# mbortolon97/6dgs

Hardware: AMD Instinct MI355X
Metric: poses/sec (higher is better)
Workload: dtype f32

## Files before the change

### 6dgs_amd/_lib.py

```python
from __future__ import annotations

import ctypes as C
import os

_HERE = os.path.dirname(os.path.abspath(__file__))
LIB_PATH = os.path.join(_HERE, "csrc", "lib6dgs_hip.so")
if os.environ.get("SIXDGS_LIB"):
    LIB_PATH = os.path.abspath(os.environ["SIXDGS_LIB"])

vp = C.c_void_p
i64 = C.c_int64
i32 = C.c_int
sz = C.c_size_t


PROFILE_SLOTS = 128
ABI_VERSION = 10


class Profile(C.Structure):
    _fields_ = [("count", i32), ("start", vp * PROFILE_SLOTS), ("stop", vp * PROFILE_SLOTS),
                ("flops", C.c_double * PROFILE_SLOTS), ("bytes", C.c_double * PROFILE_SLOTS)]


# ... 21 lines not shown
    "sixdgs_splat_views": (i32, [vp, vp, i32, vp, vp, i32, i32, i64, vp, i32, i32, i32, i32, C.c_float, C.c_float, vp, vp, vp, vp, sz, vp]),
    "sixdgs_packed_weights_floats": (sz, []),
    "sixdgs_pack_weights": (i32, [vp] * 13 + [C.POINTER(ScorerWeights), vp]),
    "sixdgs_ray_encode": (i32, [vp, vp, vp, i64, vp, vp]),
    "sixdgs_ray_keys_workspace_bytes": (sz, [i64, i64]),
    "sixdgs_ray_keys": (i32, [vp, vp, vp, i64, C.POINTER(ScorerWeights), vp, vp, vp, sz, vp]),
    "sixdgs_ray_keys_ex": (i32, [vp, vp, vp, i64, C.POINTER(ScorerWeights), vp, vp, vp, vp, vp, vp, sz, vp, C.POINTER(Profile), i32]),
    "sixdgs_key_planes_f16_bytes": (sz, [i64]),
    "sixdgs_split_planes_f16": (i32, [vp, i64, i64, vp, vp, vp]),
    "sixdgs_score_pass1": (i32, [vp, vp, vp, i32, vp, vp, vp, i64, i32, vp, vp, sz, vp, C.POINTER(Profile), i32]),
    "sixdgs_score_pass2": (i32, [vp, vp, i32, i32, i64, i32, vp, vp, vp, vp, sz, vp, i32]),
    "sixdgs_score_backward_workspace_bytes": (sz, [i32]),
    "sixdgs_score_backward": (i32, [vp, vp, i32, vp, i64, vp, vp, vp, vp, vp, sz, vp]),
    "sixdgs_score_backward_split_workspace_bytes": (sz, [i32, i64, i32]),
    "sixdgs_score_backward_split": (i32, [vp, vp, i32, vp, i64, vp, vp, vp, vp, i32, vp, sz, vp]),
    "sixdgs_score_topk_ex": (i32, [vp, vp, vp, i32, vp, vp, vp, i64, i32, vp, vp, vp, vp, vp, sz, vp, C.POINTER(Profile), i32]),
    "sixdgs_score_select_workspace_bytes": (sz, [i64, i32, i32, i32]),
    "sixdgs_score_select": (i32, [vp, vp, vp, i32, vp, vp, vp, i64, vp, vp, i64, i32, i32, vp, vp, vp, vp, sz, vp, C.POINTER(Profile)]),
    "sixdgs_tok_attention": (i32, [vp, i64, i32, i32, i32, vp, i64, vp]),
    "sixdgs_im2col": (i32, [vp, i64, i64, i64, i64, i32, i32, i32, i32, i32, i32, vp, vp]),
    "sixdgs_u8_to_planar": (i32, [vp, i32, i64, vp, vp, vp]),
    "sixdgs_image_prep": (i32, [vp, i32, i32, i32, vp, i32, i32, i32, i32, i32, vp, vp, vp, vp]),
    "sixdgs_tok_pack_bytes": (sz, [i32, i32]),
    "sixdgs_tok_pack": (i32, [vp, i32, i32, i64, vp, vp, vp]),
    "sixdgs_tok_linear": (i32, [vp, i64, i32, i64, i32, vp, vp, C.c_float, vp, vp, vp, i32, i32, vp, i64, vp, vp, i64, vp]),
    "sixdgs_key_planes_norm_max": (i32, [vp, vp, i64, vp, vp]),
    "sixdgs_select_workspace_bytes": (sz, [i64, i32, i32, i32]),
    "sixdgs_select_candidates_workspace_bytes": (sz, [i64, i32, i32, i32]),
    "sixdgs_select_begin": (i32, [vp, vp, vp, i32, vp, vp, i64, i64, vp, vp, vp, sz, vp]),
    "sixdgs_select_sweep_plan": (i32, [vp, i32, vp, vp, i32]),
    "sixdgs_select_sweep": (i32, [vp, vp, vp, i32, vp, vp, i64, vp, vp, vp, i64, vp, vp, sz, vp, C.POINTER(Profile)]),
    "sixdgs_select_candidates": (i32, [vp, i64, i64, vp, vp, vp, i32, vp, vp, vp, i32, i32, vp, vp, vp, sz, vp]),
    "sixdgs_select_rescore": (i32, [vp, vp, i32, vp, vp, i32, vp, vp, vp, vp, i64, i32, i32, i32, vp, vp, vp, vp, sz, vp]),
    "sixdgs_select_sample_stats": (i32, [vp, vp, vp, i32, vp, vp, i64, vp, vp, sz, vp]),
    "sixdgs_select_prepare": (i32, [vp, vp, i32, i64, i64, vp, vp, vp]),
    "sixdgs_select_topk_u": (i32, [vp, i64, i64, vp, i32, i32, vp, vp, sz, vp]),
    "sixdgs_linear_splitk_workspace_bytes": (sz, [i64, i32, i32]),
    "sixdgs_linear_splitk": (i32, [vp, i64, i32, i64, vp, i64, vp, i32, i32, vp, i64, i32, vp, sz, vp, i32]),
    "sixdgs_linear_ex": (i32, [vp, i64, i32, i64, vp, i64, vp, i32, i32, vp, i64, vp, i32]),
    "sixdgs_profile_collect": (i32, [C.POINTER(Profile), C.POINTER(C.c_double), C.POINTER(C.c_double), C.POINTER(C.c_double),
                                    C.POINTER(i32)]),
    "sixdgs_linear": (i32, [vp, i64, i32, i64, vp, i64, vp, i32, i32, vp, i64, vp]),
    "sixdgs_q_proj": (i32, [vp, vp, i32, C.POINTER(ScorerWeights), vp, vp]),
    "sixdgs_score_topk_workspace_bytes": (sz, [i64, i32, i32]),
    "sixdgs_score_topk_workspace_bytes_ex": (sz, [i64, i32, i32, i32, i32]),
    "sixdgs_score_topk": (i32, [vp, vp, i32, vp, i64, i32, vp, vp, vp, vp, vp, sz, vp]),
    "sixdgs_topk_workspace_bytes": (sz, [i64, i32, i32]),
    "sixdgs_topk": (i32, [vp, i64, i32, i32, vp, vp, vp, sz, vp]),
    "sixdgs_distance_target_workspace_bytes": (sz, [i64]),
    "sixdgs_distance_target": (i32, [vp, vp, i64, vp, i32, vp, vp, vp, sz, vp]),
    "sixdgs_solve_pose": (i32, [vp, vp, i64, vp, vp, i32, vp, vp, i32, vp, vp, vp, vp, vp, vp, vp]),
    "sixdgs_solve_pose_consensus_workspace_bytes": (sz, [i32, i32]),
    "sixdgs_solve_pose_consensus": (i32, [vp, vp, i64, vp, vp, i32, vp, vp, i32, C.c_float, i32] + [vp] * 10 + [vp, sz, vp]),
}

_lib = None


def load():
    global _lib
    if _lib is not None:
        return _lib
    import torch

    if not os.path.exists(LIB_PATH):
        raise RuntimeError(
# ... 24 lines not shown
```

### 6dgs_amd/csrc/score.hip

```cpp
#include <stdlib.h>

#include <cstdlib>
#include <cstdio>
#include "gemm_kernel.h"
#include "sweep_plan.h"
#include "sweep_layout.h"

using namespace sdg;

namespace {

constexpr int kT = SIXDGS_MAX_TOKENS;
constexpr float kSqrtD = 19.595917942265423f;

struct LogitsArgs {
  const float* q;
  const int* n_tok;
  const float* key;
  float* logits;
  float* partial;
  int64_t r, ldl;
  int tiles_per_group, n_tiles, n_groups;
  int b0;
};
// ... 1207 lines not shown
    if (i + 2 < R) m = fmaxf(m, a.z);
    if (i + 3 < R) m = fmaxf(m, a.w);
  }
  if (tmax != nullptr) {
    m = sdg_wave_max(m);
    const int64_t tile = (i - 4 * sdg_lane()) >> 8;
    if (sdg_lane() == 0 && tile * 256 < R) tmax[(int64_t)img * tmax_stride + tile] = m;
  }
}

__global__ void __launch_bounds__(256) k_plane_norm_max(const char* __restrict__ planes, const float* __restrict__ inv_scale, int64_t rows,
                                                        unsigned* __restrict__ out) {
  const int lane = sdg_lane();
  const int64_t wave0 = (int64_t)blockIdx.x * 4 + sdg_wave(), nw = (int64_t)gridDim.x * 4;
  float best = 0.f;
  for (int64_t row = wave0; row < rows; row += nw) {
    float ss = 0.f;
    if (lane < 48) {
      const char* p = planes + row * kRowF + (lane >> 2) * kSlabF + (lane & 3) * 16;
      const f16x8 h = *reinterpret_cast<const f16x8*>(p), l = *reinterpret_cast<const f16x8*>(p + 64);
#pragma unroll
      for (int e = 0; e < 8; ++e) {
        const float x = (float)h[e] + (float)l[e];
        ss = __builtin_fmaf(x, x, ss);
      }
    }
    ss = sdg_wave_sum(ss);
    best = fmaxf(best, sqrtf(ss) * inv_scale[row >> 7]);
  }
  if (lane == 0 && best > 0.f) atomicMax(out, __float_as_uint(best * 1.000244140625f));
}

constexpr float kEpsPerX = 1.4e-4f, kEpsConst = 1.3e-5f;
__global__ void __launch_bounds__(kT) k_sel_bounds(const float* __restrict__ gsum, const int* __restrict__ n_tok, const float* __restrict__ valU,
                                                   const float* __restrict__ q, const float* __restrict__ key_norm_max, int topk, int k_eff,
                                                   float* __restrict__ info, const int* __restrict__ only) {
  __shared__ float smin[4], smax[4], sq[4];
  const int bl = blockIdx.x, t = threadIdx.x, M = n_tok[bl];
  if (only != nullptr && only[bl] == 0) return;
  const float g = gsum[(int64_t)bl * kT + t];
  float lo = t < M ? g : INFINITY, hi = t < M ? g : -INFINITY;
  bool bad = t < M && !(g > 0.f && g < INFINITY);
  float qn = 0.f;
  if (t < M) {
    const float4* qr = reinterpret_cast<const float4*>(q + ((int64_t)bl * kT + t) * SIXDGS_D);
    float ss = 0.f;
    for (int i = 0; i < SIXDGS_D / 4; ++i) {
      const float4 v = qr[i];
      ss = __builtin_fmaf(v.x, v.x, ss); ss = __builtin_fmaf(v.y, v.y, ss); ss = __builtin_fmaf(v.z, v.z, ss); ss = __builtin_fmaf(v.w, v.w, ss);
    }
    qn = sqrtf(ss) * 1.000244140625f;
  }
#pragma unroll
  for (int o = 32; o > 0; o >>= 1) {
    lo = fminf(lo, __shfl_xor(lo, o, 64));
    hi = fmaxf(hi, __shfl_xor(hi, o, 64));
    qn = fmaxf(qn, __shfl_xor(qn, o, 64));
  }
  const unsigned long long anybad = __ballot(bad);
  if (sdg_lane() == 0) { smin[sdg_wave()] = anybad ? NAN : lo; smax[sdg_wave()] = hi; sq[sdg_wave()] = qn; }
  __syncthreads();
  if (t == 0) {
    float flag = 0.f, thr = INFINITY, eps = 0.f, x = 0.f;
    if (M <= 0) flag = 1.f;
    else {
      float a = smin[0], b = smax[0], qm = sq[0];
      bool nan = a != a;
      for (int w = 1; w < 4; ++w) { nan = nan || smin[w] != smin[w]; a = fminf(a, smin[w]); b = fmaxf(b, smax[w]); qm = fmaxf(qm, sq[w]); }
      const float uk = valU[(int64_t)bl * topk + (k_eff - 1)];
      x = qm * key_norm_max[0] * kInvSqrtD * 1.0000002f;
      eps = x * kEpsPerX + kEpsConst;
      if (nan || !(uk >= 0.f && uk < INFINITY) || !(a > 0.f) || !(eps < 0.25f)) flag = 2.f;
      else thr = (uk * (a / b)) * ((1.f - eps) / (1.f + eps)) * 0.9999998f;
    }
    info[bl * 4 + 0] = thr;
    info[bl * 4 + 1] = flag;
    info[bl * 4 + 2] = eps;
    info[bl * 4 + 3] = x;
  }
}

__global__ void k_sel_need_exact(const int* __restrict__ total, const float* __restrict__ info, int nb, int cmax, int* __restrict__ need) {
  const int bl = blockIdx.x * blockDim.x + threadIdx.x;
  if (bl >= nb) return;
  need[bl] = (info[bl * 4 + 1] == 0.f && total[bl] > cmax) ? 1 : 0;
}

__global__ void k_sel_count(const int* __restrict__ total, const float* __restrict__ info, int nb, int* __restrict__ d_count) {
  const int bl = blockIdx.x * blockDim.x + threadIdx.x;
  if (bl >= nb) return;
  const float flag = info[bl * 4 + 1];
  d_count[bl] = flag == 1.f ? -2 : (flag != 0.f ? -1 : total[bl]);
}

template <bool WRITE>
__global__ void __launch_bounds__(256) k_sel_candidates(const float* __restrict__ U, int64_t stride, int64_t R, const float* __restrict__ info,
                                                        int64_t span, unsigned* __restrict__ counts, const unsigned* __restrict__ offs,
                                                        int64_t* __restrict__ cand, int cmax, const int* __restrict__ only,
                                                        const float* __restrict__ tmax_all) {
  __shared__ int sc[4];
  const int bl = blockIdx.y;
  if (only != nullptr && only[bl] == 0) return;
  const float thr = info[bl * 4 + 0];
  const float* u = U + (int64_t)bl * stride;
  const float* tmax = tmax_all ? tmax_all + (int64_t)bl * (stride >> 8) : nullptr;
  const int64_t i0 = (int64_t)blockIdx.x * span, i1 = min(i0 + span, R);
  unsigned run = 0;
  const unsigned base = WRITE ? offs[(int64_t)bl * gridDim.x + blockIdx.x] : 0u;
  for (int64_t c0 = i0; c0 < i1; c0 += 256) {
    if (tmax != nullptr && !(tmax[c0 >> 8] >= thr)) continue;
    const int64_t i = c0 + threadIdx.x;
    const bool in = i < i1 && u[i] >= thr;
// ... 65 lines not shown
    }
#pragma unroll
    for (int c = 0; c < 8; ++c) {
      double a = acc[c];
#pragma unroll
      for (int j = 0; j < 4; ++j) {
        const f16x8 kh = *reinterpret_cast<const f16x8*>(krow[c] + sl * kSlabF + j * 16);
        const f16x8 kl = *reinterpret_cast<const f16x8*>(krow[c] + sl * kSlabF + 64 + j * 16);
#pragma unroll
        for (int e = 0; e < 8; ++e) {
          const double h = (double)(float)kh[e], l = (double)(float)kl[e], qhh = (double)(float)qh[j][e], qll = (double)(float)ql[j][e];
          a = __builtin_fma(h, qll, a);
          a = __builtin_fma(l, qhh, a);
          a = __builtin_fma(h, qhh, a);
        }
      }
      acc[c] = a;
    }
  }
  const float cq = qinv[2 * b + (t >> 7)], ct = t < M ? ctok[(int64_t)bl * kT + t] : -INFINITY;
  const float gt = gsum[(int64_t)bl * kT + t], rgt = (t < M && gt > 0.f) ? 1.f / gt : 0.f;
#pragma unroll
  for (int c = 0; c < 8; ++c) {
    const float cfl = ((cq * kscale[c]) * kInvSqrtD) * kLog2e;
    float e = t < M ? __builtin_amdgcn_exp2f(__builtin_fmaf((float)acc[c], cfl, ct)) * rgt : 0.f;
    e = sdg_wave_sum(e);
    if (sdg_lane() == 0) red[c][sdg_wave()] = e;
  }
  __syncthreads();
  if (t < 8 && c0 + t < cmax)
    cscore[(int64_t)bl * cmax + c0 + t] = t < nc ? (red[t][0] + red[t][1]) + (red[t][2] + red[t][3]) : -INFINITY;
}

__global__ void __launch_bounds__(1024) k_sel_emit(const int64_t* __restrict__ lidx, const float* __restrict__ lval, const int64_t* __restrict__ cand,
                                                   const int* __restrict__ count, int cmax, int topk, int k_eff, int allow_fewer,
                                                   int64_t* __restrict__ idx, float* __restrict__ val, int* __restrict__ status) {
  const int bl = blockIdx.x, j = threadIdx.x;
  const int n = count[bl];
  int st = n;
  if (n == -2) st = 0;
  else if (n < 0 || n > cmax || (n < k_eff && !allow_fewer)) st = -1;
  if (allow_fewer && n >= 0 && n < k_eff) k_eff = n;
  if (j == 0) status[bl] = st;
  if (j >= topk) return;
  if (n == -2) {
    idx[(int64_t)bl * topk + j] = j < k_eff ? j : -1;
    val[(int64_t)bl * topk + j] = j < k_eff ? 0.f : NAN;
  } else if (st < 0 || j >= k_eff) {
    idx[(int64_t)bl * topk + j] = -1;
    val[(int64_t)bl * topk + j] = NAN;
  } else {
    idx[(int64_t)bl * topk + j] = cand[(int64_t)bl * cmax + lidx[(int64_t)bl * topk + j]];
    val[(int64_t)bl * topk + j] = lval[(int64_t)bl * topk + j];
  }
}

constexpr int64_t kTopkSmallMax = 1 << 17;
__global__ void __launch_bounds__(1024) k_topk_small(const float* __restrict__ scores, int64_t stride, int n, int topk, int k_eff,
                                                      int64_t* __restrict__ idx, float* __restrict__ val, const int* __restrict__ only) {
  __shared__ unsigned hist[256];
  __shared__ unsigned sel[3];
  __shared__ unsigned slot;
  __shared__ unsigned sk[1024];
  __shared__ long long si[1024];
  __shared__ int wc[2][16];
  const int b = blockIdx.x, t = threadIdx.x, lane = t & 63, wv = t >> 6;
  if (only != nullptr && only[b] == 0) return;
  const float* s = scores + (int64_t)b * stride;
  sk[t] = 0u;
  si[t] = 0x7fffffffffffffffll;
  unsigned prefix = 0u, remain = (unsigned)k_eff;
  if (k_eff > 0) {
    for (int p = 0; p < 4; ++p) {
      if (t < 256) hist[t] = 0u;
      __syncthreads();
      const unsigned hi_mask = p == 0 ? 0u : (0xffffffffu << (32 - 8 * p));
      const int shift = 24 - 8 * p;
      for (int c0 = 0; c0 < n; c0 += 8 * 1024) {
        float v8[8];
#pragma unroll
        for (int u = 0; u < 8; ++u) {
          const int i = c0 + u * 1024 + t;
          v8[u] = i < n ? s[i] : 0.f;
        }
#pragma unroll
        for (int u = 0; u < 8; ++u) {
          const int i = c0 + u * 1024 + t;
          if (c0 + u * 1024 >= n) break;
          unsigned key = 0u;
          bool act = false;
          if (i < n) {
            key = score_key(v8[u]);
            act = (key & hi_mask) == prefix;
          }
          const unsigned bin = (key >> shift) & 255u;
          const unsigned long long m = __ballot(act);
          if (m != 0ull) {
            const int leader = __ffsll((long long)m) - 1;
            const unsigned lb = (unsigned)__shfl((int)bin, leader);
            const unsigned long long same = __ballot(act && bin == lb);
            if (lane == leader) atomicAdd(&hist[lb], (unsigned)__popcll(same));
// ... 80 lines not shown
        if (w2 < wv) { og += g; oe += e; }
        tg += g;
        te += e;
      }
      __syncthreads();
      const unsigned long long below = (1ull << lane) - 1ull;
      if (gt) {
        const unsigned pos = run_g + og + (unsigned)__popcll(bg & below);
        if (pos < 1024u) { sk[pos] = key; si[pos] = (long long)i; }
      } else if (eq) {
        const unsigned re = run_e + oe + (unsigned)__popcll(be & below);
        if (re < remain && n_greater + re < 1024u) { sk[n_greater + re] = key; si[n_greater + re] = (long long)i; }
      }
      run_g += tg;
      run_e += te;
      if (run_e >= remain && run_g >= n_greater) break;
    }
    }
  }
  __syncthreads();
  for (int size = 2; size <= 1024; size <<= 1)
    for (int strd = size >> 1; strd > 0; strd >>= 1) {
      const int p = t ^ strd;
      if (p > t) {
        const bool up = (t & size) == 0;
        const unsigned ka = sk[t], kb = sk[p];
        const long long ia = si[t], ib = si[p];
        const bool a_first = ka > kb || (ka == kb && ia < ib);
        if (up ? !a_first : a_first) { sk[t] = kb; sk[p] = ka; si[t] = ib; si[p] = ia; }
      }
      __syncthreads();
    }
  if (t < topk) {
    if (t < k_eff) { idx[(int64_t)b * topk + t] = si[t]; val[(int64_t)b * topk + t] = key_score(sk[t]); }
    else { idx[(int64_t)b * topk + t] = -1; val[(int64_t)b * topk + t] = NAN; }
  }
}

struct TopkPlan {
  int nb;
  int64_t span;
  size_t off_hist, off_counts, off_offs, off_ckey, off_cidx, bytes;
};
TopkPlan topk_plan(int64_t r, int batch, int topk) {
  TopkPlan p;
  int64_t nb = sdg_cdiv(r, 256 * 16);
  if (nb > 2048) nb = 2048;
  if (nb < 1) nb = 1;
  p.nb = (int)nb;
  p.span = sdg_cdiv(sdg_cdiv(r, nb), 256) * 256;
  if (p.span < 256) p.span = 256;
  size_t o = 0;
  p.off_hist = o;   o += sdg_align((size_t)batch * 4 * 256 * sizeof(unsigned));
  p.off_counts = o; o += sdg_align((size_t)batch * nb * 2 * sizeof(unsigned));
  p.off_offs = o;   o += sdg_align((size_t)batch * nb * 2 * sizeof(unsigned));
  p.off_ckey = o;   o += sdg_align((size_t)batch * topk * sizeof(unsigned));
  p.off_cidx = o;   o += sdg_align((size_t)batch * topk * sizeof(int64_t));
  p.bytes = o;
  return p;
}

int run_topk(const float* scores, int64_t stride, int64_t r, int batch, int topk, int64_t* idx, float* val, char* ws,
             hipStream_t s, const int* only = nullptr) {
  const TopkPlan p = topk_plan(r, batch, topk);
  unsigned* hist = (unsigned*)(ws + p.off_hist);
  unsigned* counts = (unsigned*)(ws + p.off_counts);
  unsigned* offs = (unsigned*)(ws + p.off_offs);
  unsigned* ckey = (unsigned*)(ws + p.off_ckey);
  int64_t* cidx = (int64_t*)(ws + p.off_cidx);
// ... 570 lines not shown
  if (!tiles) {
    hipLaunchKernelGGL(k_sel_candidates<false>, cg, dim3(256), 0, s, u, u_stride, r, w.info, w.p.span, w.counts, w.offs, cand, max_candidates, none, u_tile_max);
    hipLaunchKernelGGL(k_sel_scan, dim3((unsigned)batch), dim3(1024), 0, s, w.counts, w.p.nbc, w.offs, w.total);
    hipLaunchKernelGGL(k_sel_candidates<true>, cg, dim3(256), 0, s, u, u_stride, r, w.info, w.p.span, w.counts, w.offs, cand, max_candidates, none, u_tile_max);
  }
  hipLaunchKernelGGL(k_sel_count, dim3((unsigned)sdg_cdiv(batch, 64)), dim3(64), 0, s, w.total, w.info, batch, d_count);
  SDG_LAUNCH_OK();
  return 0;
}

int sixdgs_select_rescore(const float* q, const int32_t* d_n_tok, int batch, const void* planes, const float* d_scale, int compact,
                          const float* ctok, const float* gsum, const int64_t* cand, const int32_t* d_count, int64_t r, int topk,
                          int max_candidates, int allow_fewer, int64_t* idx, float* val, int32_t* d_status, void* ws, size_t ws_bytes,
                          sixdgs_stream_t stream) {
  SDG_CHECK_ARG(batch >= 0 && r >= 1 && topk >= 1 && topk <= 1024 && max_candidates >= topk && (max_candidates % 8) == 0);
  if (batch == 0) return 0;
  SDG_CHECK_ARG(q && d_n_tok && planes && d_scale && ctok && gsum && cand && d_count && idx && val && d_status && ws &&
                ((uintptr_t)planes % 16) == 0 && ((uintptr_t)q % 16) == 0 && ((uintptr_t)ws % 256) == 0);
  hipStream_t s = sdg_stream(stream);
  const int cmax = max_candidates;
  SelectWs w;
  if (!select_ws(ws, ws_bytes, cmax, batch, topk, cmax, &w, false)) return SIXDGS_E_WORKSPACE;
  const int k_eff = (int)(r < topk ? r : topk);
  select_q_planes(q, batch, w, s);
  hipLaunchKernelGGL(k_sel_rescore, dim3((unsigned)(cmax / 8), (unsigned)batch), dim3(kT), 0, s, w.qplanes, w.qinv, (const char*)planes, d_scale,
                     d_n_tok, 0, ctok, gsum, cand, d_count, cmax, compact, w.cscore);
  const int st = run_topk(w.cscore, cmax, cmax, batch, topk, w.lidx, w.lval, w.topk_ws, s);
  if (st) return st;
  hipLaunchKernelGGL(k_sel_emit, dim3((unsigned)batch), dim3(1024), 0, s, w.lidx, w.lval, cand, d_count, cmax, topk, k_eff, allow_fewer, idx, val, d_status);
  SDG_LAUNCH_OK();
  return 0;
}

size_t sixdgs_score_select_workspace_bytes(int64_t r, int batch, int topk, int max_candidates) {
  if (batch < 1) batch = 1;
  const size_t stride = (size_t)sdg_cdiv(r > 0 ? r : 1, 256) * 256;
  return sdg_align(sixdgs_select_workspace_bytes(r, batch, topk, max_candidates)) +
         (size_t)batch * (2 * sdg_align(kT * sizeof(float)) + sdg_align(stride * sizeof(float)) + sdg_align(stride / 256 * sizeof(float)) +
                          sdg_align((size_t)max_candidates * sizeof(int64_t)) + 256);
}

int sixdgs_score_select(const float* q, const int32_t* d_n_tok, const int32_t* h_n_tok, int batch, const void* key_planes,
                        const float* d_key_scale, const float* d_key_norm_max, int64_t r, const void* sample_planes, const float* d_sample_scale,
                        int64_t r_sample, int topk, int max_candidates, int64_t* idx, float* val, int32_t* d_status, void* ws, size_t ws_bytes,
                        sixdgs_stream_t stream, sixdgs_profile* prof) {
  SDG_CHECK_ARG(r >= 1 && r_sample >= 1 && r_sample <= r && batch >= 0 && topk >= 1 && topk <= 1024 && max_candidates >= topk &&
                max_candidates <= (1 << 20) && (max_candidates % 8) == 0);
  if (batch == 0) return 0;
  SDG_CHECK_ARG(q && d_n_tok && d_key_norm_max && idx && val && d_status && ws && ((uintptr_t)ws % 256) == 0);
  int64_t bg = batch > 4096 ? 4096 : batch;
  while (bg >= 1 && sixdgs_score_select_workspace_bytes(r, (int)bg, topk, max_candidates) > ws_bytes) --bg;
  if (bg < 1) return SIXDGS_E_WORKSPACE;
  bg = sdg_cdiv(batch, sdg_cdiv(batch, bg));
  const size_t stride = (size_t)sdg_cdiv(r, 256) * 256;
  const size_t stage = sdg_align(sixdgs_select_workspace_bytes(r, (int)bg, topk, max_candidates));
  char* base = (char*)ws + stage;
  float* ctok = (float*)base;                        base += (size_t)bg * sdg_align(kT * sizeof(float));
  float* gsum = (float*)base;                        base += (size_t)bg * sdg_align(kT * sizeof(float));
  float* u = (float*)base;                           base += (size_t)bg * sdg_align(stride * sizeof(float));
  float* utm = (float*)base;                         base += (size_t)bg * sdg_align(stride / 256 * sizeof(float));
  int64_t* cand = (int64_t*)base;                    base += (size_t)bg * sdg_align((size_t)max_candidates * sizeof(int64_t));
  int32_t* count = (int32_t*)base;
  for (int b0 = 0; b0 < batch; b0 += (int)bg) {
    const int nb = (int)((batch - b0) < bg ? (batch - b0) : bg);
    const float* qg = q + (int64_t)b0 * kT * SIXDGS_D;
    const int32_t* ng = d_n_tok + b0;
    int st = sixdgs_select_begin(qg, ng, h_n_tok ? h_n_tok + b0 : nullptr, nb, sample_planes, d_sample_scale, r_sample, r, ctok, gsum, ws, stage, stream);
    if (st) return st;
    st = sixdgs_select_sweep(qg, ng, h_n_tok ? h_n_tok + b0 : nullptr, nb, key_planes, d_key_scale, r, ctok, gsum, u, (int64_t)stride, utm, ws, stage,
                             stream, prof);
    if (st) return st;
    st = sixdgs_select_candidates(u, (int64_t)stride, r, utm, qg, ng, nb, gsum, d_key_norm_max, nullptr, topk, max_candidates, cand, count, ws, stage, stream);
    if (st) return st;
    st = sixdgs_select_rescore(qg, ng, nb, key_planes, d_key_scale, 0, ctok, gsum, cand, count, r, topk, max_candidates, 0,
                               idx + (int64_t)b0 * topk, val + (int64_t)b0 * topk, d_status + b0, ws, stage, stream);
    if (st) return st;
  }
  return 0;
}

}
```

### 6dgs_amd/ops.py

```python
from __future__ import annotations

import ctypes as C
import functools
import os
import threading
from typing import Optional, Tuple

import torch

from . import _lib
from ._lib import Profile, ScorerWeights, check

D = 384
MMA_DEFAULT, MMA_F32, MMA_BF16X6, MMA_F16X3, MMA_F16X3_L32 = -1, 0, 1, 2, 3
F16_MODES = (MMA_F16X3, MMA_F16X3_L32)
MMA_LIBRARY_DEFAULT = MMA_F16X3
_mma_mode = MMA_DEFAULT


def set_mma_mode(mode: int):
    global _mma_mode
    assert mode in (MMA_DEFAULT, MMA_F32, MMA_BF16X6, MMA_F16X3, MMA_F16X3_L32)
    _mma_mode = mode

# ... 688 lines not shown
                                   _p(workspace), workspace.numel(), _stream(), profile.ref if profile is not None else None,
                                   _mma_mode), "score_topk")
    return idx, val, scores, stats


MAX_TOPK = 1024


def check_topk(k, what: str = "rays_to_output") -> int:
    if isinstance(k, bool) or int(k) != k or not 1 <= int(k) <= MAX_TOPK:
        raise ValueError(f"6dgs_amd: {what} = {k!r}: the top-k takes 1 <= k <= MAX_TOPK = {MAX_TOPK}")
    return int(k)


SELECT_MAX_CANDIDATES = 4096
SELECT_SAMPLE_STRIDE = 16
SELECT_SAMPLE_STRIDE_LARGE = 32
SELECT_LARGE_RAYS = 16_000_000
SELECT_SAMPLE_STRIDE_HUGE = 64
SELECT_HUGE_RAYS = 32_000_000
SELECT_MIN_RAYS = 1 << 20
_select_enabled = True


def set_select_enabled(on: bool):
    global _select_enabled
    _select_enabled = bool(on)


def select_enabled() -> bool:
    return _select_enabled


@_on_device
def select_sample_indices(r: int, device, stride: Optional[int] = None) -> torch.Tensor:
    if stride is None:
        stride = SELECT_SAMPLE_STRIDE_HUGE if r >= SELECT_HUGE_RAYS else (SELECT_SAMPLE_STRIDE_LARGE if r >= SELECT_LARGE_RAYS else SELECT_SAMPLE_STRIDE)
    n = r // stride
    i = torch.arange(n, dtype=torch.int64, device=device)
    return i * stride + (((i * 2654435761) & 0xFFFFFFFF) >> 13) % stride


@_on_device
def key_norm_max(planes: torch.Tensor, scale: torch.Tensor, out: Optional[torch.Tensor] = None) -> torch.Tensor:
    _need_gpu(planes, scale, out)
    if planes.shape[1] != 1536:
        raise RuntimeError("6dgs_amd: key_norm_max needs scaled fp16 key planes (MMA_F16X3)")
    if out is None:
        out = torch.zeros(1, device=planes.device)
    check(_lib.load().sixdgs_key_planes_norm_max(_p(planes), _p(scale), planes.shape[0], _p(out), _stream()), "key_planes_norm_max")
    return out


def score_select_workspace_bytes(r: int, batch: int, topk: int = 100, max_candidates: int = SELECT_MAX_CANDIDATES) -> int:
    return int(_lib.load().sixdgs_score_select_workspace_bytes(int(r), int(batch), int(topk), int(max_candidates)))


def select_sweep_plan(n_tok_host, batch: Optional[int] = None):
    lib = _lib.load()
    b = len(n_tok_host) if n_tok_host is not None else int(batch)
    h_n = (C.c_int32 * b)(*[int(v) for v in n_tok_host]) if n_tok_host is not None else None
    cap = max(1, b)
    slots, imgs = (C.c_int32 * cap)(), (C.c_int32 * cap)()
    n = lib.sixdgs_select_sweep_plan(h_n, b, slots, imgs, cap)
    if n < 0:
        check(n, "select_sweep_plan")
# ... 352 lines not shown
```

### include/sixdgs.h

```cpp
#ifndef SIXDGS_H
#define SIXDGS_H

#include <stddef.h>
#include <stdint.h>

#ifdef __cplusplus
extern "C" {
#endif

#define SIXDGS_ABI_VERSION 10
#define SIXDGS_E_BADARG (-1)
#define SIXDGS_E_WORKSPACE (-2)
#define SIXDGS_E_UNSUPPORTED (-3)

#define SIXDGS_D 384
#define SIXDGS_RAY_IN 141
#define SIXDGS_RAY_IN_PAD 144
#define SIXDGS_HID 512
#define SIXDGS_TOK_IN 398
#define SIXDGS_MAX_TOKENS 256

typedef void* sixdgs_stream_t;

#define SIXDGS_MMA_DEFAULT (-1)
// ... 153 lines not shown
                       size_t ws_bytes, sixdgs_stream_t stream, sixdgs_profile* prof, int mma_mode);
int sixdgs_score_pass2(const float* row_stats, const int32_t* d_n_tok, int batch, int used_planes, int64_t r, int topk,
                       float* scores, int64_t* idx, float* val, void* ws, size_t ws_bytes, sixdgs_stream_t stream, int mma_mode);
size_t sixdgs_score_backward_workspace_bytes(int batch);
int sixdgs_score_backward(const float* q, const int32_t* d_n_tok, int batch, const float* key , int64_t r,
                          const float* row_stats, const float* g, float* dq, float* dk, void* ws, size_t ws_bytes, sixdgs_stream_t stream);
size_t sixdgs_score_backward_split_workspace_bytes(int batch, int64_t r, int ray_groups);
int sixdgs_score_backward_split(const float* q, const int32_t* d_n_tok, int batch, const float* key , int64_t r,
                                const float* row_stats, const float* g, float* dq, float* dk, int ray_groups, void* ws, size_t ws_bytes,
                                sixdgs_stream_t stream);
size_t sixdgs_score_select_workspace_bytes(int64_t r, int batch, int topk, int max_candidates);
int sixdgs_key_planes_norm_max(const void* planes, const float* d_scale, int64_t rows, float* d_norm_max, sixdgs_stream_t stream);
size_t sixdgs_select_workspace_bytes(int64_t r, int batch, int topk, int max_candidates);
size_t sixdgs_select_candidates_workspace_bytes(int64_t r, int batch, int topk, int max_candidates);
int sixdgs_select_sweep_plan(const int32_t* h_n_tok, int batch, int32_t* slots_per_launch, int32_t* images_per_launch, int max_launches);
int sixdgs_select_begin(const float* q, const int32_t* d_n_tok, const int32_t* h_n_tok, int batch, const void* sample_planes, const float* d_sample_scale,
                        int64_t r_sample, int64_t r_total, float* ctok, float* gsum, void* ws, size_t ws_bytes, sixdgs_stream_t stream);
int sixdgs_select_sample_stats(const float* q, const int32_t* d_n_tok, const int32_t* h_n_tok, int batch, const void* sample_planes, const float* d_sample_scale,
                               int64_t r_sample, float* row_stats , void* ws, size_t ws_bytes, sixdgs_stream_t stream);
int sixdgs_select_prepare(const float* row_stats, const int32_t* d_n_tok, int batch, int64_t r_sample, int64_t r_total, float* ctok, float* gsum,
                          sixdgs_stream_t stream);
int sixdgs_select_topk_u(const float* u, int64_t u_stride, int64_t r, const float* u_tile_max , int batch, int topk, float* val ,
                         void* ws, size_t ws_bytes, sixdgs_stream_t stream);
int sixdgs_select_sweep(const float* q, const int32_t* d_n_tok, const int32_t* h_n_tok, int batch, const void* key_planes,
                        const float* d_key_scale, int64_t r, const float* ctok, float* gsum, float* u, int64_t u_stride, float* u_tile_max,
                        void* ws, size_t ws_bytes, sixdgs_stream_t stream, sixdgs_profile* prof);
int sixdgs_select_candidates(const float* u, int64_t u_stride, int64_t r, const float* u_tile_max , const float* q, const int32_t* d_n_tok, int batch, const float* gsum,
                             const float* d_key_norm_max, const float* d_uk ,
                             int topk, int max_candidates, int64_t* cand, int32_t* d_count, void* ws, size_t ws_bytes, sixdgs_stream_t stream);
int sixdgs_select_rescore(const float* q, const int32_t* d_n_tok, int batch, const void* planes, const float* d_scale, int compact,
                          const float* ctok, const float* gsum, const int64_t* cand, const int32_t* d_count, int64_t r, int topk,
                          int max_candidates, int allow_fewer, int64_t* idx, float* val, int32_t* d_status, void* ws, size_t ws_bytes,
                          sixdgs_stream_t stream);
int sixdgs_score_select(const float* q, const int32_t* d_n_tok, const int32_t* h_n_tok ,
                        int batch, const void* key_planes, const float* d_key_scale, const float* d_key_norm_max, int64_t r,
                        const void* sample_planes, const float* d_sample_scale, int64_t r_sample, int topk, int max_candidates, int64_t* idx ,
                        float* val , int32_t* d_status , void* ws, size_t ws_bytes, sixdgs_stream_t stream,
                        sixdgs_profile* prof);
size_t sixdgs_topk_workspace_bytes(int64_t r, int batch, int topk);
int sixdgs_topk(const float* scores, int64_t r, int batch, int topk, int64_t* idx, float* val, void* ws,
                size_t ws_bytes, sixdgs_stream_t stream);

size_t sixdgs_distance_target_workspace_bytes(int64_t r);
int sixdgs_distance_target(const float* rays_ori, const float* rays_dir, int64_t r, const float* d_pose, int n_tokens,
                           float* target , float* d_sum, void* ws, size_t ws_bytes, sixdgs_stream_t stream);

int sixdgs_solve_pose(const float* rays_ori, const float* rays_dir, int64_t r, const int64_t* idx ,
                      const float* val , int k, const float* up , const float* gt_c2w ,
                      int batch, float* c2w, int32_t* status, float* w_final, int32_t* n_kept, float* centre ,
                      float* errors, sixdgs_stream_t stream);

size_t sixdgs_solve_pose_consensus_workspace_bytes(int batch, int k);
int sixdgs_solve_pose_consensus(const float* rays_ori, const float* rays_dir, int64_t r, const int64_t* idx ,
                                const float* val , int k, const float* up , const float* gt_c2w ,
                                int batch, float tau, int prior, float* c2w, int32_t* status, float* w_final, int32_t* n_kept,
                                float* centre , float* errors, float* support, int32_t* n_inliers, float* rms,
                                int32_t* winner, void* ws, size_t ws_bytes, sixdgs_stream_t stream);

#ifdef __cplusplus
}
#endif
#endif
```

Before: 73.03.

## Fuse select candidate topk, bounds and compaction into one per-batch kernel

Adds a fused select tail. One kernel per batch row runs the small top-k over tile maxima or scores, computes the bounds, and compacts candidates, retrying without tiles when they overflow. A second kernel merges candidate top-k with emit. This replaces the separate candidate and rescore launch sequences in score_select, cutting kernel launches and global round trips. The cost is one 1024-thread block per batch row with large LDS use, which may limit parallelism on large R.

Result: no change. 73.11 (median of 6 runs) (+0.1%).

```diff
diff --git a/6dgs_amd/_lib.py b/6dgs_amd/_lib.py
--- a/6dgs_amd/_lib.py
+++ b/6dgs_amd/_lib.py
@@ -77,6 +77,7 @@
     "sixdgs_select_sweep": (i32, [vp, vp, vp, i32, vp, vp, i64, vp, vp, vp, i64, vp, vp, sz, vp, C.POINTER(Profile)]),
     "sixdgs_select_candidates": (i32, [vp, i64, i64, vp, vp, vp, i32, vp, vp, vp, i32, i32, vp, vp, vp, sz, vp]),
     "sixdgs_select_rescore": (i32, [vp, vp, i32, vp, vp, i32, vp, vp, vp, vp, i64, i32, i32, i32, vp, vp, vp, vp, sz, vp]),
+    "sixdgs_select_tail": (i32, [vp, i64, i64, vp, vp, vp, i32, vp, vp, vp, vp, vp, i32, i32, vp, vp, vp, vp, vp, vp, sz, vp]),
     "sixdgs_select_sample_stats": (i32, [vp, vp, vp, i32, vp, vp, i64, vp, vp, sz, vp]),
     "sixdgs_select_prepare": (i32, [vp, vp, i32, i64, i64, vp, vp, vp]),
     "sixdgs_select_topk_u": (i32, [vp, i64, i64, vp, i32, i32, vp, vp, sz, vp]),
diff --git a/6dgs_amd/csrc/score.hip b/6dgs_amd/csrc/score.hip
--- a/6dgs_amd/csrc/score.hip
+++ b/6dgs_amd/csrc/score.hip
@@ -1263,13 +1263,15 @@
 }
 
 constexpr float kEpsPerX = 1.4e-4f, kEpsConst = 1.3e-5f;
-__global__ void __launch_bounds__(kT) k_sel_bounds(const float* __restrict__ gsum, const int* __restrict__ n_tok, const float* __restrict__ valU,
-                                                   const float* __restrict__ q, const float* __restrict__ key_norm_max, int topk, int k_eff,
-                                                   float* __restrict__ info, const int* __restrict__ only) {
-  __shared__ float smin[4], smax[4], sq[4];
-  const int bl = blockIdx.x, t = threadIdx.x, M = n_tok[bl];
-  if (only != nullptr && only[bl] == 0) return;
-  const float g = gsum[(int64_t)bl * kT + t];
+struct SelBoundsLds { float smin[4], smax[4], sq[4]; };
+__device__ __forceinline__ void sel_bounds_wg(int bl, const float* __restrict__ gsum, const int* __restrict__ n_tok, const float* __restrict__ valU,
+                                              const float* __restrict__ q, const float* __restrict__ key_norm_max, int topk, int k_eff,
+                                              float* __restrict__ info, SelBoundsLds& L) {
+  float (&smin)[4] = L.smin;
+  float (&smax)[4] = L.smax;
+  float (&sq)[4] = L.sq;
+  const int t = threadIdx.x, M = min(n_tok[bl], t < kT ? kT : 0);
+  const float g = t < kT ? gsum[(int64_t)bl * kT + t] : 0.f;
   float lo = t < M ? g : INFINITY, hi = t < M ? g : -INFINITY;
   bool bad = t < M && !(g > 0.f && g < INFINITY);
   float qn = 0.f;
@@ -1289,7 +1291,7 @@
     qn = fmaxf(qn, __shfl_xor(qn, o, 64));
   }
   const unsigned long long anybad = __ballot(bad);
-  if (sdg_lane() == 0) { smin[sdg_wave()] = anybad ? NAN : lo; smax[sdg_wave()] = hi; sq[sdg_wave()] = qn; }
+  if (sdg_lane() == 0 && sdg_wave() < 4) { smin[sdg_wave()] = anybad ? NAN : lo; smax[sdg_wave()] = hi; sq[sdg_wave()] = qn; }
   __syncthreads();
   if (t == 0) {
     float flag = 0.f, thr = INFINITY, eps = 0.f, x = 0.f;
@@ -1309,6 +1311,14 @@
     info[bl * 4 + 2] = eps;
     info[bl * 4 + 3] = x;
   }
+}
+__global__ void __launch_bounds__(kT) k_sel_bounds(const float* __restrict__ gsum, const int* __restrict__ n_tok, const float* __restrict__ valU,
+                                                   const float* __restrict__ q, const float* __restrict__ key_norm_max, int topk, int k_eff,
+                                                   float* __restrict__ info, const int* __restrict__ only) {
+  __shared__ SelBoundsLds L;
+  const int bl = blockIdx.x;
+  if (only != nullptr && only[bl] == 0) return;
+  sel_bounds_wg(bl, gsum, n_tok, valU, q, key_norm_max, topk, k_eff, info, L);
 }
 
 __global__ void k_sel_need_exact(const int* __restrict__ total, const float* __restrict__ info, int nb, int cmax, int* __restrict__ need) {
@@ -1440,10 +1450,10 @@
     cscore[(int64_t)bl * cmax + c0 + t] = t < nc ? (red[t][0] + red[t][1]) + (red[t][2] + red[t][3]) : -INFINITY;
 }
 
-__global__ void __launch_bounds__(1024) k_sel_emit(const int64_t* __restrict__ lidx, const float* __restrict__ lval, const int64_t* __restrict__ cand,
-                                                   const int* __restrict__ count, int cmax, int topk, int k_eff, int allow_fewer,
-                                                   int64_t* __restrict__ idx, float* __restrict__ val, int* __restrict__ status) {
-  const int bl = blockIdx.x, j = threadIdx.x;
+__device__ __forceinline__ void sel_emit_wg(int bl, const int64_t* __restrict__ lidx, const float* __restrict__ lval, const int64_t* __restrict__ cand,
+                                            const int* __restrict__ count, int cmax, int topk, int k_eff, int allow_fewer,
+                                            int64_t* __restrict__ idx, float* __restrict__ val, int* __restrict__ status) {
+  const int j = threadIdx.x;
   const int n = count[bl];
   int st = n;
   if (n == -2) st = 0;
@@ -1462,19 +1472,30 @@
     val[(int64_t)bl * topk + j] = lval[(int64_t)bl * topk + j];
   }
 }
+__global__ void __launch_bounds__(1024) k_sel_emit(const int64_t* __restrict__ lidx, const float* __restrict__ lval, const int64_t* __restrict__ cand,
+                                                   const int* __restrict__ count, int cmax, int topk, int k_eff, int allow_fewer,
+                                                   int64_t* __restrict__ idx, float* __restrict__ val, int* __restrict__ status) {
+  sel_emit_wg(blockIdx.x, lidx, lval, cand, count, cmax, topk, k_eff, allow_fewer, idx, val, status);
+}
 
 constexpr int64_t kTopkSmallMax = 1 << 17;
-__global__ void __launch_bounds__(1024) k_topk_small(const float* __restrict__ scores, int64_t stride, int n, int topk, int k_eff,
-                                                      int64_t* __restrict__ idx, float* __restrict__ val, const int* __restrict__ only) {
-  __shared__ unsigned hist[256];
-  __shared__ unsigned sel[3];
-  __shared__ unsigned slot;
-  __shared__ unsigned sk[1024];
-  __shared__ long long si[1024];
-  __shared__ int wc[2][16];
-  const int b = blockIdx.x, t = threadIdx.x, lane = t & 63, wv = t >> 6;
-  if (only != nullptr && only[b] == 0) return;
-  const float* s = scores + (int64_t)b * stride;
+struct TopkSmallLds {
+  unsigned hist[256];
+  unsigned sel[3];
+  unsigned slot;
+  unsigned sk[1024];
+  long long si[1024];
+  int wc[2][16];
+};
+__device__ __forceinline__ void topk_small_wg(const float* __restrict__ s, int n, int topk, int k_eff, int64_t* __restrict__ idx, float* __restrict__ val,
+                                              TopkSmallLds& L) {
+  unsigned (&hist)[256] = L.hist;
+  unsigned (&sel)[3] = L.sel;
+  unsigned& slot = L.slot;
+  unsigned (&sk)[1024] = L.sk;
+  long long (&si)[1024] = L.si;
+  int (&wc)[2][16] = L.wc;
+  const int t = threadIdx.x, lane = t & 63, wv = t >> 6;
   sk[t] = 0u;
   si[t] = 0x7fffffffffffffffll;
   unsigned prefix = 0u, remain = (unsigned)k_eff;
@@ -1621,9 +1642,118 @@
       __syncthreads();
     }
   if (t < topk) {
-    if (t < k_eff) { idx[(int64_t)b * topk + t] = si[t]; val[(int64_t)b * topk + t] = key_score(sk[t]); }
-    else { idx[(int64_t)b * topk + t] = -1; val[(int64_t)b * topk + t] = NAN; }
-  }
+    if (t < k_eff) { idx[t] = si[t]; val[t] = key_score(sk[t]); }
+    else { idx[t] = -1; val[t] = NAN; }
+  }
+}
+__global__ void __launch_bounds__(1024) k_topk_small(const float* __restrict__ scores, int64_t stride, int n, int topk, int k_eff,
+                                                      int64_t* __restrict__ idx, float* __restrict__ val, const int* __restrict__ only) {
+  __shared__ TopkSmallLds L;
+  const int b = blockIdx.x;
+  if (only != nullptr && only[b] == 0) return;
+  topk_small_wg(scores + (int64_t)b * stride, n, topk, k_eff, idx + (int64_t)b * topk, val + (int64_t)b * topk, L);
+}
+
+struct SelCompactLds {
+  int tiles[1024];
+  unsigned scan[17];
+  int wc[4][16];
+};
+__device__ __forceinline__ unsigned sel_compact_wg(const float* __restrict__ u, int64_t R, const float* __restrict__ tmax, float thr,
+                                                   int64_t* __restrict__ cand, int cmax, SelCompactLds& L) {
+  const int t = threadIdx.x, lane = t & 63, wv = t >> 6;
+  const int64_t nt = (R + 255) >> 8;
+  unsigned run = 0u;
+  for (int64_t t0 = 0; t0 < nt; t0 += 1024) {
+    const int64_t tile = t0 + t;
+    const bool q = tile < nt && (tmax == nullptr || tmax[tile] >= thr);
+    unsigned nq;
+    const unsigned at = sdg_block_exclusive_scan<unsigned, 16>(q ? 1u : 0u, L.scan, &nq);
+    if (q) L.tiles[at] = t;
+    __syncthreads();
+    for (unsigned v0 = 0; v0 < nq * 256u; v0 += 4096u) {
+      int64_t i[4];
+      float x[4];
+#pragma unroll
+      for (int j = 0; j < 4; ++j) {
+        const unsigned v = v0 + (unsigned)j * 1024u + (unsigned)t;
+        i[j] = v < nq * 256u ? ((t0 + L.tiles[v >> 8]) << 8) + (int64_t)(v & 255u) : R;
+        x[j] = i[j] < R ? u[i[j]] : 0.f;
+      }
+      unsigned long long bm[4];
+#pragma unroll
+      for (int j = 0; j < 4; ++j) {
+        bm[j] = __ballot(i[j] < R && x[j] >= thr);
+        if (lane == 0) L.wc[j][wv] = __popcll(bm[j]);
+      }
+      __syncthreads();
+      unsigned before[4] = {0u, 0u, 0u, 0u}, tot = 0u;
+#pragma unroll
+      for (int j = 0; j < 4; ++j) {
+        before[j] = tot;
+#pragma unroll
+        for (int w2 = 0; w2 < 16; ++w2) {
+          const unsigned c = (unsigned)L.wc[j][w2];
+          if (w2 < wv) before[j] += c;
+          tot += c;
+        }
+      }
+      __syncthreads();
+#pragma unroll
+      for (int j = 0; j < 4; ++j)
+        if (i[j] < R && x[j] >= thr) {
+          const unsigned pos = run + before[j] + (unsigned)__popcll(bm[j] & ((1ull << lane) - 1ull));
+          if (pos < (unsigned)cmax) cand[pos] = i[j];
+        }
+      run = run + tot < run ? 0xffffffffu : run + tot;
+    }
+  }
+  return run;
+}
+
+__global__ void __launch_bounds__(1024) k_sel_tail(const float* __restrict__ U, int64_t stride, int64_t R, const float* __restrict__ tmax_all, int tiles,
+                                                   const float* __restrict__ q, const int* __restrict__ n_tok, const float* __restrict__ gsum,
+                                                   const float* __restrict__ key_norm_max, int topk, int k_eff, int cmax, int64_t* __restrict__ idxU,
+                                                   float* __restrict__ valU, float* __restrict__ info, int64_t* __restrict__ cand,
+                                                   int* __restrict__ total, int* __restrict__ d_count) {
+  __shared__ TopkSmallLds LT;
+  __shared__ SelBoundsLds LB;
+  __shared__ SelCompactLds LC;
+  const int bl = blockIdx.x;
+  const float* u = U + (int64_t)bl * stride;
+  const float* tmax = tmax_all ? tmax_all + (int64_t)bl * (stride >> 8) : nullptr;
+  int64_t* iu = idxU + (int64_t)bl * topk;
+  float* vu = valU + (int64_t)bl * topk;
+  int64_t* cd = cand + (int64_t)bl * cmax;
+  unsigned n = 0u;
+  for (int pass = 0; pass < 2; ++pass) {
+    const bool from_tiles = tiles != 0 && pass == 0;
+    __syncthreads();
+    if (from_tiles) topk_small_wg(tmax, (int)((R + 255) >> 8), topk, topk, iu, vu, LT);
+    else topk_small_wg(u, (int)R, topk, k_eff, iu, vu, LT);
+    __syncthreads();
+    sel_bounds_wg(bl, gsum, n_tok, valU, q, key_norm_max, topk, from_tiles ? topk : k_eff, info, LB);
+    __syncthreads();
+    const float thr = info[bl * 4 + 0], flag = info[bl * 4 + 1];
+    n = sel_compact_wg(u, R, tmax, thr, cd, cmax, LC);
+    if (!(from_tiles && flag == 0.f && n > (unsigned)cmax)) break;
+  }
+  if (threadIdx.x == 0) {
+    const float flag = info[bl * 4 + 1];
+    const int tot = (int)min(n, 0x7fffffffu);
+    total[bl] = tot;
+    d_count[bl] = flag == 1.f ? -2 : (flag != 0.f ? -1 : tot);
+  }
+}
+
+__global__ void __launch_bounds__(1024) k_sel_pick(const float* __restrict__ cscore, const int64_t* __restrict__ cand, const int* __restrict__ count,
+                                                   int cmax, int topk, int k_eff, int allow_fewer, int64_t* __restrict__ lidx, float* __restrict__ lval,
+                                                   int64_t* __restrict__ idx, float* __restrict__ val, int* __restrict__ status) {
+  __shared__ TopkSmallLds LT;
+  const int bl = blockIdx.x;
+  topk_small_wg(cscore + (int64_t)bl * cmax, cmax, topk, min(cmax, topk), lidx + (int64_t)bl * topk, lval + (int64_t)bl * topk, LT);
+  __syncthreads();
+  sel_emit_wg(bl, lidx, lval, cand, count, cmax, topk, k_eff, allow_fewer, idx, val, status);
 }
 
 struct TopkPlan {
@@ -2260,6 +2390,46 @@
   return 0;
 }
 
+static bool select_tail_fused() {
+  const char* e = getenv("SIXDGS_SELECT_TAIL");
+  return !(e && atoi(e) == 0);
+}
+
+int sixdgs_select_tail(const float* u, int64_t u_stride, int64_t r, const float* u_tile_max, const float* q, const int32_t* d_n_tok, int batch,
+                       const void* key_planes, const float* d_key_scale, const float* ctok, const float* gsum, const float* d_key_norm_max, int topk,
+                       int max_candidates, int64_t* cand, int32_t* d_count, int64_t* idx, float* val, int32_t* d_status, void* ws, size_t ws_bytes,
+                       sixdgs_stream_t stream) {
+  SDG_CHECK_ARG(batch >= 0 && r >= 1 && u_stride >= r && topk >= 1 && topk <= 1024 && max_candidates >= topk && (max_candidates % 8) == 0);
+  if (batch == 0) return 0;
+  SDG_CHECK_ARG(u && q && d_n_tok && key_planes && d_key_scale && ctok && gsum && d_key_norm_max && cand && d_count && idx && val && d_status && ws &&
+                ((uintptr_t)ws % 256) == 0 && ((uintptr_t)q % 16) == 0 && ((uintptr_t)key_planes % 16) == 0);
+  const int cmax = max_candidates;
+  const int64_t nt = sdg_cdiv(r, 256);
+  const bool tiles = u_tile_max && nt >= 2 * (int64_t)topk;
+  SDG_CHECK_ARG(!u_tile_max || ((u_stride % 256) == 0 && u_stride >= nt * 256));
+  static const bool small_ok = getenv("SIXDGS_TOPK_SMALL") == nullptr || atoi(getenv("SIXDGS_TOPK_SMALL")) != 0;
+  const bool fused = select_tail_fused() && small_ok && cmax <= kTopkSmallMax && r <= (int64_t)1 << 30 && (tiles ? nt : r) <= kTopkSmallMax;
+  if (!fused) {
+    const int st = sixdgs_select_candidates(u, u_stride, r, u_tile_max, q, d_n_tok, batch, gsum, d_key_norm_max, nullptr, topk, cmax, cand, d_count, ws,
+                                            ws_bytes, stream);
+    if (st) return st;
+    return sixdgs_select_rescore(q, d_n_tok, batch, key_planes, d_key_scale, 0, ctok, gsum, cand, d_count, r, topk, cmax, 0, idx, val, d_status, ws,
+                                 ws_bytes, stream);
+  }
+  hipStream_t s = sdg_stream(stream);
+  SelectWs w, wr;
+  if (!select_ws(ws, ws_bytes, r, batch, topk, cmax, &w, false) || !select_ws(ws, ws_bytes, cmax, batch, topk, cmax, &wr, false)) return SIXDGS_E_WORKSPACE;
+  const int k_eff = (int)(r < topk ? r : topk);
+  hipLaunchKernelGGL(k_sel_tail, dim3((unsigned)batch), dim3(1024), 0, s, u, u_stride, r, u_tile_max, tiles ? 1 : 0, q, d_n_tok, gsum, d_key_norm_max, topk,
+                     k_eff, cmax, w.idxU, w.valU, w.info, cand, w.total, d_count);
+  select_q_planes(q, batch, wr, s);
+  hipLaunchKernelGGL(k_sel_rescore, dim3((unsigned)(cmax / 8), (unsigned)batch), dim3(kT), 0, s, wr.qplanes, wr.qinv, (const char*)key_planes, d_key_scale,
+                     d_n_tok, 0, ctok, gsum, cand, d_count, cmax, 0, wr.cscore);
+  hipLaunchKernelGGL(k_sel_pick, dim3((unsigned)batch), dim3(1024), 0, s, wr.cscore, cand, d_count, cmax, topk, k_eff, 0, wr.lidx, wr.lval, idx, val, d_status);
+  SDG_LAUNCH_OK();
+  return 0;
+}
+
 size_t sixdgs_score_select_workspace_bytes(int64_t r, int batch, int topk, int max_candidates) {
   if (batch < 1) batch = 1;
   const size_t stride = (size_t)sdg_cdiv(r > 0 ? r : 1, 256) * 256;
@@ -2298,11 +2468,9 @@
     st = sixdgs_select_sweep(qg, ng, h_n_tok ? h_n_tok + b0 : nullptr, nb, key_planes, d_key_scale, r, ctok, gsum, u, (int64_t)stride, utm, ws, stage,
                              stream, prof);
     if (st) return st;
-    st = sixdgs_select_candidates(u, (int64_t)stride, r, utm, qg, ng, nb, gsum, d_key_norm_max, nullptr, topk, max_candidates, cand, count, ws, stage, stream);
+    st = sixdgs_select_tail(u, (int64_t)stride, r, utm, qg, ng, nb, key_planes, d_key_scale, ctok, gsum, d_key_norm_max, topk, max_candidates, cand, count,
+                            idx + (int64_t)b0 * topk, val + (int64_t)b0 * topk, d_status + b0, ws, stage, stream);
     if (st) return st;
-    st = sixdgs_select_rescore(qg, ng, nb, key_planes, d_key_scale, 0, ctok, gsum, cand, count, r, topk, max_candidates, 0,
-                               idx + (int64_t)b0 * topk, val + (int64_t)b0 * topk, d_status + b0, ws, stage, stream);
-    if (st) return st;
   }
   return 0;
 }
diff --git a/6dgs_amd/ops.py b/6dgs_amd/ops.py
--- a/6dgs_amd/ops.py
+++ b/6dgs_amd/ops.py
@@ -744,6 +744,14 @@
     return _select_enabled
 
 
+def set_select_tail(fused: bool):
+    os.environ["SIXDGS_SELECT_TAIL"] = "1" if fused else "0"
+
+
+def select_tail_fused() -> bool:
+    return os.environ.get("SIXDGS_SELECT_TAIL", "1") != "0"
+
+
 @_on_device
 def select_sample_indices(r: int, device, stride: Optional[int] = None) -> torch.Tensor:
     if stride is None:
diff --git a/include/sixdgs.h b/include/sixdgs.h
--- a/include/sixdgs.h
+++ b/include/sixdgs.h
@@ -209,6 +209,10 @@
                           const float* ctok, const float* gsum, const int64_t* cand, const int32_t* d_count, int64_t r, int topk,
                           int max_candidates, int allow_fewer, int64_t* idx, float* val, int32_t* d_status, void* ws, size_t ws_bytes,
                           sixdgs_stream_t stream);
+int sixdgs_select_tail(const float* u, int64_t u_stride, int64_t r, const float* u_tile_max , const float* q, const int32_t* d_n_tok, int batch,
+                       const void* key_planes, const float* d_key_scale, const float* ctok, const float* gsum, const float* d_key_norm_max, int topk,
+                       int max_candidates, int64_t* cand, int32_t* d_count, int64_t* idx, float* val, int32_t* d_status, void* ws, size_t ws_bytes,
+                       sixdgs_stream_t stream);
 int sixdgs_score_select(const float* q, const int32_t* d_n_tok, const int32_t* h_n_tok ,
                         int batch, const void* key_planes, const float* d_key_scale, const float* d_key_norm_max, int64_t r,
                         const void* sample_planes, const float* d_sample_scale, int64_t r_sample, int topk, int max_candidates, int64_t* idx ,
```
